# IvanPopov/video-flow-ml

Hardware: AMD Instinct MI355X
Metric: flow-fields/sec @1080p seq5 MOF_sintel (higher is better)
Workload: dtype mixed (per-layer MFMA count, f32 accumulate): {"corr": 1, "update_block.encoder.convf1": 1, "update_block.encoder.convf2": 1, "update_block.gru.convq1.iter": "2a", "update_block.gru.convzr1.iter": 1, "update_block.gru.convzr2.iter": 1, "update_block.mask.0": 1, "update_block.mask.2": 1, "update_bloc

## Files before the change

### video-flow-ml_amd/vfml/csrc/enc_conv.hip

```cpp
#include "conv_split_common.h"

namespace {

constexpr int EC_C = 64;
constexpr int EC_TH = 4, EC_TW = 32;
constexpr int EC_PR = EC_TH + 2, EC_PW = EC_TW + 2;
constexpr int EC_PIX = 272;
constexpr int EC_PATCH = EC_PR * EC_PW * EC_PIX;
constexpr int EC_VLD = EC_C + 4;
constexpr int EC_LDS = EC_PATCH;
constexpr int EC_K = 9 * EC_C;
constexpr int EC_NS = EC_K / 32;
static_assert(EC_TH * EC_TW * EC_VLD * 4 <= EC_PATCH, "the result tile fits where the patch was");

struct EncConvArgs {
  const char* in;
  const _Float16* whi; const _Float16* wlo;
  const float* bias;
  float* out; int ldo;
  double* stats_part;
  int ld_in, n, H, W, tiles_x, tiles_y;
  float w_inv;
};

__global__ __launch_bounds__(256, 2) void enc_conv3x3_c64_kernel(const EncConvArgs a) {
  extern __shared__ __attribute__((aligned(16))) char smem[];
  float* sV = reinterpret_cast<float*>(smem);

  const int t = threadIdx.x, lane = t & 63;
  const int wave = __builtin_amdgcn_readfirstlane(t >> 6);
  const int r4 = lane & 15, u4 = lane >> 4;
  const int tiles_img = a.tiles_x * a.tiles_y;
  const int total = a.n * tiles_img;

  h16x8 bh[EC_NS], bl[EC_NS];
  static_for<EC_NS>([&](auto sc) {
    constexpr int s = decltype(sc)::value;
    bh[s] = *reinterpret_cast<const h16x8*>(a.whi + (16 * wave + r4) * EC_K + s * 32 + u4 * 8);
    bl[s] = *reinterpret_cast<const h16x8*>(a.wlo + (16 * wave + r4) * EC_K + s * 32 + u4 * 8);
  });
  f32x4 bias4 = {0.f, 0.f, 0.f, 0.f};
  if (a.bias) bias4 = *reinterpret_cast<const f32x4*>(a.bias + 16 * wave + 4 * u4);

  for (int tile = blockIdx.x; tile < total; tile += gridDim.x) {
    const int img = tile / tiles_img, tl = tile - img * tiles_img;
    const int ty = tl / a.tiles_x, tx = tl - ty * a.tiles_x;
    const int oy0 = ty * EC_TH, ox0 = tx * EC_TW;

    constexpr int NPC = EC_PR * EC_PW * 16;
    constexpr int NPT = (NPC + 255) / 256;
    const __amdgpu_buffer_rsrc_t rin = __builtin_amdgcn_make_buffer_rsrc(
        const_cast<char*>(a.in) + (int64_t)img * a.H * a.W * a.ld_in * 4, 0, a.H * a.W * a.ld_in * 4, 0x00020000);
    u32x4 pv[NPT];
    static_for<NPT>([&](auto qc) {
      constexpr int q = decltype(qc)::value;
      const int c = min(t + 256 * q, NPC - 1);
      const int p = c >> 4, piece = c & 15;
      const int py = p / EC_PW, px = p - py * EC_PW;
      const int iy = oy0 - 1 + py, ix = ox0 - 1 + px;
      const bool ok = (unsigned)iy < (unsigned)a.H && (unsigned)ix < (unsigned)a.W;
      pv[q] = bload16(rin, ok ? ((iy * a.W + ix) * a.ld_in) * 4 + piece * 16 : (int)0x80000000);
    });
    __syncthreads();
    static_for<NPT>([&](auto qc) {
      constexpr int q = decltype(qc)::value;
      const int c = t + 256 * q;
      if (c < NPC) *reinterpret_cast<u32x4*>(smem + (c >> 4) * EC_PIX + (c & 15) * 16) = pv[q];
    });
    __syncthreads();

    f32x4 acc[8];
#pragma unroll
    for (int m = 0; m < 8; ++m) acc[m] = f32x4{0.f, 0.f, 0.f, 0.f};
    const char* al = smem + r4 * EC_PIX + u4 * 32;
    static_for<2>([&](auto hc) {
      constexpr int mh = decltype(hc)::value;
      static_for<EC_NS>([&](auto sc) {
        constexpr int s = decltype(sc)::value;
        constexpr int cb = s / 9, ky = (s % 9) / 3, kx = s % 3;
#pragma unroll
        for (int mm = 0; mm < 4; ++mm) {
          const int m = 4 * mh + mm;
          const char* p = al + (((m >> 1) + ky) * EC_PW + 16 * (m & 1) + kx) * EC_PIX + cb * 128;
          const h16x8 ah = *reinterpret_cast<const h16x8*>(p);
          const h16x8 alo = *reinterpret_cast<const h16x8*>(p + 16);
          acc[m] = __builtin_amdgcn_mfma_f32_16x16x32_f16(bh[s], ah, acc[m], 0, 0, 0);
          acc[m] = __builtin_amdgcn_mfma_f32_16x16x32_f16(bl[s], ah, acc[m], 0, 0, 0);
          acc[m] = __builtin_amdgcn_mfma_f32_16x16x32_f16(bh[s], alo, acc[m], 0, 0, 0);
        }
        if constexpr (s % 3 == 2) __builtin_amdgcn_sched_barrier(0);
      });
      __builtin_amdgcn_sched_barrier(0);
    });

    __syncthreads();
#pragma unroll
    for (int m = 0; m < 8; ++m) {
      f32x4 v;
#pragma unroll
      for (int e = 0; e < 4; ++e) v[e] = acc[m][e] * a.w_inv + bias4[e];
      const int row = m >> 1, col = 16 * (m & 1) + r4;
      const int oy = oy0 + row, ox = ox0 + col;
      *reinterpret_cast<f32x4*>(&sV[(row * EC_TW + col) * EC_VLD + 16 * wave + 4 * u4]) = v;
      if (oy < a.H && ox < a.W)
        *reinterpret_cast<f32x4*>(a.out + (((int64_t)img * a.H + oy) * a.W + ox) * a.ldo + 16 * wave + 4 * u4) = v;
    }
    if (a.stats_part) {
      __syncthreads();
      const int row = t >> 6, ch = t & 63;
      const int oy = oy0 + row;
      if (oy < a.H) {
        double s1 = 0.0, s2 = 0.0;
        for (int x = 0; x < EC_TW; ++x) {
          float f = sV[(row * EC_TW + x) * EC_VLD + ch], g;
          asm("v_mov_b32 %0, %1" : "=v"(g) : "v"(f));
          const double v = (double)g;
          s1 += v;
          s2 += v * v;
        }
        const int64_t chunk = (((int64_t)img * a.H + oy) * a.W + ox0) >> 5;
        double* o = a.stats_part + (chunk * EC_C + ch) * 2;
        o[0] = s1;
        o[1] = s2;
      }
    }
  }
}

}

extern "C" int vfml_conv3x3_c64(const float* in, int ld_in, int n, int h, int w, const void* w_hi, const void* w_lo, int kp,
                                float w_scale, const float* bias, float* out, int ldo, double* stats_part, void* stream) {
  VFML_REQUIRE(in && w_hi && w_lo && out && n > 0 && h > 0 && w > 0, "vfml_conv3x3_c64: bad argument");
  VFML_REQUIRE(w % EC_TW == 0, "vfml_conv3x3_c64: the image width must be a multiple of %d (got %d)", EC_TW, w);
  VFML_REQUIRE(kp == EC_K && w_scale > 0.f, "vfml_conv3x3_c64: weight planes [64][%d] (VFML_KORDER_CBLOCK), got row pitch %d", EC_K, kp);
  VFML_REQUIRE((reinterpret_cast<uintptr_t>(in) & 31u) == 0 && ld_in >= EC_C && ld_in % 8 == 0 && vfml_aligned16(w_hi) &&
                   vfml_aligned16(w_lo) && vfml_aligned16(bias) && vfml_aligned16(out) && ldo >= EC_C && ldo % 4 == 0 &&
                   (reinterpret_cast<uintptr_t>(stats_part) & 7u) == 0,
               "vfml_conv3x3_c64: a 32-byte aligned split-row input (ld_in %% 8 == 0), 16-byte aligned weights / bias / output "
               "(ldo %% 4 == 0)");
  EncConvArgs a;
  a.in = reinterpret_cast<const char*>(in); a.ld_in = ld_in;
  a.whi = reinterpret_cast<const _Float16*>(w_hi); a.wlo = reinterpret_cast<const _Float16*>(w_lo);
  a.bias = bias; a.out = out; a.ldo = ldo; a.stats_part = stats_part;
  a.n = n; a.H = h; a.W = w; a.tiles_x = w / EC_TW; a.tiles_y = (h + EC_TH - 1) / EC_TH;
  a.w_inv = 1.0f / w_scale;
  const int64_t total = (int64_t)n * a.tiles_x * a.tiles_y;
  VFML_REQUIRE(total < (1ll << 31) && (int64_t)h * w * ld_in * 4 < (1ll << 31), "vfml_conv3x3_c64: an image of the input must stay below 2 GiB");
  const int grid = (int)(total < 512 ? total : 512);
  hipLaunchKernelGGL(enc_conv3x3_c64_kernel, dim3(grid), dim3(256), EC_LDS, reinterpret_cast<hipStream_t>(stream), a);
  return vfml_check_launch("vfml_conv3x3_c64");
}
```

Measured before the change: 47.21.

## Double-buffer encoder conv input by channel block with async DMA and swizzled LDS

Splits the input patch into two 32-channel halves loaded with direct global-to-LDS DMA into separate buffers. The second half, and the next tile's first half, are fetched while MFMAs consume the current half. The LDS layout is swizzled, and fragment reads are software-pipelined a few groups ahead to hide LDS latency. This removes the register-staged load plus barrier stall before each tile's compute, at the cost of more LDS and more complex edge masking.

Result: no change. 47.34 (median of 6 runs) (+0.3%).

```diff
diff --git a/video-flow-ml_amd/vfml/csrc/enc_conv.hip b/video-flow-ml_amd/vfml/csrc/enc_conv.hip
--- a/video-flow-ml_amd/vfml/csrc/enc_conv.hip
+++ b/video-flow-ml_amd/vfml/csrc/enc_conv.hip
@@ -5,13 +5,20 @@
 constexpr int EC_C = 64;
 constexpr int EC_TH = 4, EC_TW = 32;
 constexpr int EC_PR = EC_TH + 2, EC_PW = EC_TW + 2;
-constexpr int EC_PIX = 272;
-constexpr int EC_PATCH = EC_PR * EC_PW * EC_PIX;
+constexpr int EC_LW = 40;
+constexpr int EC_RP = EC_LW / 8;
+constexpr int EC_NPC = EC_PR * EC_RP;
+constexpr int EC_NPI = (EC_NPC + 3) / 4;
+constexpr int EC_HALF = EC_NPC * 1024;
 constexpr int EC_VLD = EC_C + 4;
-constexpr int EC_LDS = EC_PATCH;
+constexpr int EC_VHALF = 64 * EC_VLD * 4;
+constexpr int EC_A0 = 0, EC_A1 = EC_HALF, EC_S = 2 * EC_HALF;
+constexpr int EC_LDS = EC_S + EC_VHALF;
 constexpr int EC_K = 9 * EC_C;
 constexpr int EC_NS = EC_K / 32;
-static_assert(EC_TH * EC_TW * EC_VLD * 4 <= EC_PATCH, "the result tile fits where the patch was");
+constexpr int EC_AHEAD = 2;
+static_assert(EC_VHALF <= EC_HALF, "the result tile's second half fits in the second channel block's buffer");
+static_assert(EC_LDS <= 80 * 1024, "two workgroups per CU");
 
 struct EncConvArgs {
   const char* in;
@@ -25,7 +32,6 @@
 
 __global__ __launch_bounds__(256, 2) void enc_conv3x3_c64_kernel(const EncConvArgs a) {
   extern __shared__ __attribute__((aligned(16))) char smem[];
-  float* sV = reinterpret_cast<float*>(smem);
 
   const int t = threadIdx.x, lane = t & 63;
   const int wave = __builtin_amdgcn_readfirstlane(t >> 6);
@@ -42,58 +48,90 @@
   f32x4 bias4 = {0.f, 0.f, 0.f, 0.f};
   if (a.bias) bias4 = *reinterpret_cast<const f32x4*>(a.bias + 16 * wave + 4 * u4);
 
-  for (int tile = blockIdx.x; tile < total; tile += gridDim.x) {
+  const int sw = (4 * wave + (lane >> 4)) & 7;
+  const int l8 = lane >> 3;
+  const int voff0 = l8 * a.ld_in * 4 + ((lane & 7) ^ swz16(sw)) * 16;
+  constexpr int EC_BAD = (int)0xF0000000;
+  auto issue_half = [&](int tl_, int cb, int dst) {
+    const int img = tl_ / tiles_img, tl = tl_ - img * tiles_img;
+    const int ty = tl / a.tiles_x, tx = tl - ty * a.tiles_x;
+    const int oy0 = ty * EC_TH, ox0 = tx * EC_TW;
+    const __amdgpu_buffer_rsrc_t rin = __builtin_amdgcn_make_buffer_rsrc(
+        const_cast<char*>(a.in) + ((int64_t)img * a.H * a.W - 1) * a.ld_in * 4, 0, (int)(((unsigned)(a.H * a.W) + 1u) * a.ld_in * 4u),
+        0x00020000);
+    const int badL = ox0 == 0 && l8 == 0 ? EC_BAD : 0;
+    const int badR = l8 >= EC_PW - 8 * (EC_RP - 1) || (l8 == 1 && ox0 + EC_TW >= a.W) ? EC_BAD : 0;
+#pragma unroll
+    for (int i = 0; i < EC_NPI; ++i) {
+      const int pc = 4 * i + wave;
+      if (4 * i + 3 < EC_NPC || pc < EC_NPC) {
+        const int py = pc / EC_RP, g = pc - py * EC_RP;
+        const int iy = oy0 - 1 + py;
+        const int rowok = -(int)((unsigned)iy < (unsigned)a.H);
+        const int vo = voff0 | (~rowok & EC_BAD) | (badL & -(int)(g == 0)) | (badR & -(int)(g == EC_RP - 1));
+        const int so = (((iy * a.W + ox0 + 8 * g) * a.ld_in) * 4 + cb * 128) & rowok;
+        dma16(rin, vo, so, smem + dst + pc * 1024);
+      }
+    }
+  };
+
+  int abase[6], abase_lo[6];
+#pragma unroll
+  for (int k = 0; k < 6; ++k) {
+    const int c = k < 3 ? k : k + 5;
+    abase[k] = (r4 + c) * 128 + ((2 * u4) ^ swz16(((r4 + c) >> 1) & 7)) * 16;
+    abase_lo[k] = abase[k] ^ 16;
+  }
+
+  f32x4 acc[8];
+  auto k_steps = [&](auto cbc, int buf) {
+    constexpr int cb = decltype(cbc)::value;
+    constexpr int NG = 72, RING = EC_AHEAD + 1;
+    h16x8 fh[RING], fl[RING];
+    auto read_group = [&](auto gc) {
+      constexpr int g = decltype(gc)::value;
+      constexpr int m = 4 * (g / 36) + g % 4, tap = (g % 36) / 4, ky = tap / 3, kx = tap % 3;
+      constexpr int C = ((m >> 1) + ky) * EC_LW + 16 * (m & 1) + kx;
+      constexpr int c = C & 15;
+      static_assert(c < 3 || (c >= 8 && c < 11), "six fragment bases");
+      constexpr int k = c < 3 ? c : c - 5;
+      fh[g % RING] = *reinterpret_cast<const h16x8*>(smem + abase[k] + (buf + (C >> 4) * 2048));
+      fl[g % RING] = *reinterpret_cast<const h16x8*>(smem + abase_lo[k] + (buf + (C >> 4) * 2048));
+    };
+    static_for<EC_AHEAD>([&](auto gc) { read_group(gc); });
+    __builtin_amdgcn_sched_barrier(0);
+    static_for<NG>([&](auto gc) {
+      constexpr int g = decltype(gc)::value;
+      constexpr int m = 4 * (g / 36) + g % 4, s = cb * 9 + (g % 36) / 4;
+      if constexpr (g + EC_AHEAD < NG) read_group(std::integral_constant<int, g + EC_AHEAD>{});
+      __builtin_amdgcn_sched_barrier(0);
+      acc[m] = __builtin_amdgcn_mfma_f32_16x16x32_f16(bh[s], fh[g % RING], acc[m], 0, 0, 0);
+      acc[m] = __builtin_amdgcn_mfma_f32_16x16x32_f16(bl[s], fh[g % RING], acc[m], 0, 0, 0);
+      acc[m] = __builtin_amdgcn_mfma_f32_16x16x32_f16(bh[s], fl[g % RING], acc[m], 0, 0, 0);
+      __builtin_amdgcn_sched_barrier(0);
+    });
+  };
+
+  int tile = blockIdx.x;
+  if (tile < total) issue_half(tile, 0, EC_A0);
+  asm volatile("s_waitcnt vmcnt(0)" ::: "memory");
+  for (; tile < total; tile += gridDim.x) {
     const int img = tile / tiles_img, tl = tile - img * tiles_img;
     const int ty = tl / a.tiles_x, tx = tl - ty * a.tiles_x;
     const int oy0 = ty * EC_TH, ox0 = tx * EC_TW;
 
-    constexpr int NPC = EC_PR * EC_PW * 16;
-    constexpr int NPT = (NPC + 255) / 256;
-    const __amdgpu_buffer_rsrc_t rin = __builtin_amdgcn_make_buffer_rsrc(
-        const_cast<char*>(a.in) + (int64_t)img * a.H * a.W * a.ld_in * 4, 0, a.H * a.W * a.ld_in * 4, 0x00020000);
-    u32x4 pv[NPT];
-    static_for<NPT>([&](auto qc) {
-      constexpr int q = decltype(qc)::value;
-      const int c = min(t + 256 * q, NPC - 1);
-      const int p = c >> 4, piece = c & 15;
-      const int py = p / EC_PW, px = p - py * EC_PW;
-      const int iy = oy0 - 1 + py, ix = ox0 - 1 + px;
-      const bool ok = (unsigned)iy < (unsigned)a.H && (unsigned)ix < (unsigned)a.W;
-      pv[q] = bload16(rin, ok ? ((iy * a.W + ix) * a.ld_in) * 4 + piece * 16 : (int)0x80000000);
-    });
-    __syncthreads();
-    static_for<NPT>([&](auto qc) {
-      constexpr int q = decltype(qc)::value;
-      const int c = t + 256 * q;
-      if (c < NPC) *reinterpret_cast<u32x4*>(smem + (c >> 4) * EC_PIX + (c & 15) * 16) = pv[q];
-    });
-    __syncthreads();
-
-    f32x4 acc[8];
+    lds_barrier();
+    issue_half(tile, 1, EC_A1);
 #pragma unroll
     for (int m = 0; m < 8; ++m) acc[m] = f32x4{0.f, 0.f, 0.f, 0.f};
-    const char* al = smem + r4 * EC_PIX + u4 * 32;
-    static_for<2>([&](auto hc) {
-      constexpr int mh = decltype(hc)::value;
-      static_for<EC_NS>([&](auto sc) {
-        constexpr int s = decltype(sc)::value;
-        constexpr int cb = s / 9, ky = (s % 9) / 3, kx = s % 3;
-#pragma unroll
-        for (int mm = 0; mm < 4; ++mm) {
-          const int m = 4 * mh + mm;
-          const char* p = al + (((m >> 1) + ky) * EC_PW + 16 * (m & 1) + kx) * EC_PIX + cb * 128;
-          const h16x8 ah = *reinterpret_cast<const h16x8*>(p);
-          const h16x8 alo = *reinterpret_cast<const h16x8*>(p + 16);
-          acc[m] = __builtin_amdgcn_mfma_f32_16x16x32_f16(bh[s], ah, acc[m], 0, 0, 0);
-          acc[m] = __builtin_amdgcn_mfma_f32_16x16x32_f16(bl[s], ah, acc[m], 0, 0, 0);
-          acc[m] = __builtin_amdgcn_mfma_f32_16x16x32_f16(bh[s], alo, acc[m], 0, 0, 0);
-        }
-        if constexpr (s % 3 == 2) __builtin_amdgcn_sched_barrier(0);
-      });
-      __builtin_amdgcn_sched_barrier(0);
-    });
+    k_steps(std::integral_constant<int, 0>{}, EC_A0);
+    asm volatile("s_waitcnt vmcnt(0)" ::: "memory");
+    lds_barrier();
+    if (tile + (int)gridDim.x < total) issue_half(tile + (int)gridDim.x, 0, EC_A0);
+    k_steps(std::integral_constant<int, 1>{}, EC_A1);
+    asm volatile("s_waitcnt vmcnt(0)" ::: "memory");
+    lds_barrier();
 
-    __syncthreads();
 #pragma unroll
     for (int m = 0; m < 8; ++m) {
       f32x4 v;
@@ -101,18 +139,20 @@
       for (int e = 0; e < 4; ++e) v[e] = acc[m][e] * a.w_inv + bias4[e];
       const int row = m >> 1, col = 16 * (m & 1) + r4;
       const int oy = oy0 + row, ox = ox0 + col;
-      *reinterpret_cast<f32x4*>(&sV[(row * EC_TW + col) * EC_VLD + 16 * wave + 4 * u4]) = v;
+      float* sV = reinterpret_cast<float*>(smem + (m < 4 ? EC_S : EC_A1));
+      *reinterpret_cast<f32x4*>(&sV[((row & 1) * EC_TW + col) * EC_VLD + 16 * wave + 4 * u4]) = v;
       if (oy < a.H && ox < a.W)
         *reinterpret_cast<f32x4*>(a.out + (((int64_t)img * a.H + oy) * a.W + ox) * a.ldo + 16 * wave + 4 * u4) = v;
     }
     if (a.stats_part) {
-      __syncthreads();
-      const int row = t >> 6, ch = t & 63;
+      lds_barrier();
+      const int row = wave, ch = t & 63;
       const int oy = oy0 + row;
+      const float* sV = reinterpret_cast<const float*>(smem + (row < 2 ? EC_S : EC_A1));
       if (oy < a.H) {
         double s1 = 0.0, s2 = 0.0;
         for (int x = 0; x < EC_TW; ++x) {
-          float f = sV[(row * EC_TW + x) * EC_VLD + ch], g;
+          float f = sV[((row & 1) * EC_TW + x) * EC_VLD + ch], g;
           asm("v_mov_b32 %0, %1" : "=v"(g) : "v"(f));
           const double v = (double)g;
           s1 += v;
@@ -148,6 +188,7 @@
   const int64_t total = (int64_t)n * a.tiles_x * a.tiles_y;
   VFML_REQUIRE(total < (1ll << 31) && (int64_t)h * w * ld_in * 4 < (1ll << 31), "vfml_conv3x3_c64: an image of the input must stay below 2 GiB");
   const int grid = (int)(total < 512 ? total : 512);
+  if (const int rc = vfml_lds_cap(reinterpret_cast<const void*>(&enc_conv3x3_c64_kernel), EC_LDS, "vfml_conv3x3_c64")) return rc;
   hipLaunchKernelGGL(enc_conv3x3_c64_kernel, dim3(grid), dim3(256), EC_LDS, reinterpret_cast<hipStream_t>(stream), a);
   return vfml_check_launch("vfml_conv3x3_c64");
 }
```
